# Hunger-Prevails/3D-Pose-Estimation-with-Previleged-Information

Measured on AMD Instinct MI355X. Metric: crops/sec (fwd+bwd) ResNet-50 pose head, 256x256 bs=64/GPU, higher is better.
Workload: dtype f32 (3xbf16 split, 6 products, f32 accumulate); 1 GPU; depthnet resnet50 pose head, 256x256 crops, batch 64/GPU, full step: fwd + soft-argmax + SmoothL1 + bwd + RCCL grad all-reduce + clip + Adam; global_batch=64, parallelism=dp1, dist_world_size=1, wgrad_stream_runs_beside_launch_stream=True

## Files before the change

3d-pose-estimation-with-previleged-information_amd/_lib.py:

```python
import ctypes
import os

_HERE = os.path.dirname(os.path.abspath(__file__))
LIB_PATH = os.environ.get('P3D_LIB') or os.path.join(_HERE, 'csrc', 'libp3d_hip.so')
HEADER_PATH = os.path.join(os.path.dirname(_HERE), 'include', 'p3d_hip.h')


class P3DError(RuntimeError):
    pass


class ConvDesc(ctypes.Structure):
    _fields_ = [(n, ctypes.c_int32) for n in
                ('N', 'C', 'H', 'W', 'K', 'R', 'S', 'stride', 'pad', 'dil', 'Ho', 'Wo', 'c_total', 'c_offset',
                 'accumulate', 'reserved')]


class FoldJob(ctypes.Structure):
    _fields_ = [(n, ctypes.c_void_p) for n in ('w', 'conv_bias', 'gamma', 'beta', 'mean', 'var', 'out', 'bias_out')] + \
               [(n, ctypes.c_int32) for n in ('K', 'C', 'RS', 'c_offset', 'c_total', 'kind')] + [('eps', ctypes.c_float), ('reserved', ctypes.c_int32)]


_i32, _i64, _f32 = ctypes.c_int32, ctypes.c_int64, ctypes.c_float
_ptr, _sz = ctypes.c_void_p, ctypes.c_size_t
# ... 25 lines not shown
    'p3d_fx_conv_fwd_infer_supported': (_i32, [_desc, _i32]),
    'p3d_fx_conv_fwd_infer_workspace_bytes': (_sz, [_desc]),
    'p3d_fx_conv_fwd_infer': (_i32, [_desc, _ptr, _ptr, _ptr, _sz, _ptr, _ptr, _i32, _ptr, _ptr, _sz, _ptr]),
    'p3d_fx_conv_fwd_infer_masked_supported': (_i32, [_desc]),
    'p3d_fx_conv_fwd_infer_masked': (_i32, [_desc, _ptr, _ptr, _sz, _ptr, _ptr, _ptr, _ptr, _i32, _ptr, _ptr, _sz, _ptr]),
    'p3d_stem_tail_infer': (_i32, [_ptr, _ptr, _ptr, _i32, _i32, _i32, _i32, _ptr]),
    'p3d_hblock_workspace_bytes': (_i32, [_ptr, _ptr, _ptr]),
    'p3d_hblock_fwd': (_i32, [_ptr, _ptr, _ptr, _sz, _ptr]),
    'p3d_hblock_bwd': (_i32, [_ptr, _ptr, _ptr, _sz, _ptr, _sz, _ptr, _ptr]),
    'p3d_fx_act_image_bytes': (_sz, [_i32, _i32, _i32]),
    'p3d_fx_act_image': (_i32, [_i32, _ptr, _ptr, _ptr, _i32, _ptr, _i32, _i32, _i32, _ptr]),
    'p3d_fx_conv_img_workspace_bytes': (_sz, [_ptr, _i32]),
    'p3d_fx_conv_img_supported': (_i32, [_ptr]),
    'p3d_fx_conv_fwd_img': (_i32, [_ptr, _ptr, _ptr, _ptr, _ptr, _ptr, _ptr, _sz, _ptr]),
    'p3d_fx_conv_dgrad_img': (_i32, [_ptr, _ptr, _ptr, _ptr, _ptr, _ptr, _sz, _ptr]),
    'p3d_fx_conv_wgrad_img': (_i32, [_ptr, _ptr, _ptr, _ptr, _ptr, _ptr, _sz, _ptr]),
    'p3d_stem_supported': (_i32, [_i32] * 5),
    'p3d_stem_image_bytes': (_sz, [_i32] * 3),
    'p3d_stem_weight_image_bytes': (_sz, [_i32]),
    'p3d_stem_workspace_bytes': (_sz, [_i32] * 4),
    'p3d_stem_image': (_i32, [_ptr, _ptr, _i32, _i32, _i32, _i32, _ptr]),
    'p3d_stem_weight_image': (_i32, [_ptr, _i32, _i32, _ptr, _ptr, _sz, _ptr]),
    'p3d_stem_fwd': (_i32, [_ptr, _ptr, _ptr, _i32, _i32, _i32, _i32, _i32, _ptr]),
    'p3d_stem_wgrad': (_i32, [_ptr, _ptr, _ptr, _i32, _i32, _i32, _i32, _i32, _i32, _ptr, _sz, _ptr]),
    'p3d_stem_masked_supported': (_i32, [_i32] * 5),
    'p3d_stem_image_masked': (_i32, [_ptr, _ptr, _ptr, _i32, _i32, _i32, _i32, _ptr]),
    'p3d_stem_fwd_masked': (_i32, [_ptr, _ptr, _ptr, _ptr, _i32, _i32, _i32, _i32, _i32, _ptr]),
    'p3d_stem_wgrad_masked': (_i32, [_ptr, _ptr, _ptr, _ptr, _i32, _i32, _i32, _i32, _i32, _i32, _ptr, _sz, _ptr]),
    'p3d_profile_enable': (_i32, [_i32]),
    'p3d_profile_collect': (_i32, [ctypes.POINTER(ctypes.c_double), ctypes.POINTER(ctypes.c_double), ctypes.POINTER(ctypes.c_int64)]),
# ... 96 lines not shown
```

3d-pose-estimation-with-previleged-information_amd/csrc/p3d_block.hip:

```cpp
#include "p3d_common.h"
#include "p3d_fx.h"
#include <vector>
#include <mutex>

namespace p3d {

using f32x4 = float __attribute__((ext_vector_type(4)));

constexpr int CLOSE_MAX_SPLIT = 64;
constexpr int FIN_CH = 16, FIN_MAX_LANES = 64;
static inline unsigned fin_threads(int rows) { return rows > 64 ? 1024u : 256u; }
constexpr int BLOCK_MIN_M = 64;
static bool block_conv_ok(const p3d_conv_desc* d, bool main_chain) {
    return fx_fwd_applies(d, BLOCK_MIN_M) && fx_dgrad_applies(d, BLOCK_MIN_M) && fx_wgrad_applies(d, BLOCK_MIN_M) && (d->Ho * d->Wo) % 4 == 0 &&
           (d->H * d->W) % 4 == 0 && d->C % 16 == 0 && d->K % 16 == 0 && !(main_chain && fx_dgrad_has_dead_classes(d));
}

__device__ __forceinline__ void blk_sum3(double& a, double& b, double& c, double* red ) {
    a = wave_sum(a); b = wave_sum(b); c = wave_sum(c);
    const int w = threadIdx.x >> 6;
    if ((threadIdx.x & 63) == 0) { red[w] = a; red[4 + w] = b; red[8 + w] = c; }
    __syncthreads();
    a = red[0] + red[1] + red[2] + red[3];
    b = red[4] + red[5] + red[6] + red[7];
// ... 798 lines not shown
}

int32_t p3d_fx_conv_dgrad_img(const p3d_conv_desc* d, const void* dy_img, const float* w, const void* wimgT, float* dx, void* workspace, size_t workspace_bytes,
                              void* stream) {
    P3D_REQUIRE(d && dy_img && w && dx, "fx_conv_dgrad_img: null argument");
    P3D_REQUIRE(fx_dgrad_applies(d, 32) && d->K % 16 == 0 && (d->Ho * d->Wo) % 4 == 0, "fx_conv_dgrad_img: shape outside the x3 kernels");
    FxFuse f{};
    f.act_img = dy_img; f.wimg = wimgT;
    ProfScope ps(1, d, (hipStream_t)stream);
    fx_count(1, d);
    if (fx_dgrad_has_dead_classes(d) && !d->accumulate)
        if (hipMemsetAsync(dx, 0, (size_t)d->N * d->C * d->H * d->W * sizeof(float), (hipStream_t)stream) != hipSuccess) { set_error("fx_conv_dgrad_img: memset failed"); return P3D_ELAUNCH; }
    return fx_conv_dgrad(d, nullptr, w, dx, workspace, workspace_bytes, &f, (hipStream_t)stream);
}

int32_t p3d_fx_conv_wgrad_img(const p3d_conv_desc* d, const void* dy_img, const float* x, const void* x_img, float* dw, void* workspace, size_t workspace_bytes,
                              void* stream) {
    P3D_REQUIRE(d && dy_img && (x || x_img) && dw, "fx_conv_wgrad_img: null argument");
    P3D_REQUIRE(fx_wgrad_applies(d, 32) && d->K % 16 == 0 && (!x_img || d->C % 16 == 0), "fx_conv_wgrad_img: shape outside the x3 kernels");
    const int splits = fx_wgrad_splits(d, x_img != nullptr);
    const size_t need = (size_t)splits * d->K * d->C * d->R * d->S * sizeof(float);
    if (!workspace || workspace_bytes < need) { set_error("fx_conv_wgrad_img: workspace %zu B < required %zu B", workspace_bytes, need); return P3D_EWORKSPACE; }
    FxFuse f{};
    f.dy_img = dy_img; f.x_img = x_img;
    ProfScope ps(2, d, (hipStream_t)stream);
    fx_count(2, d);
    if (int32_t e = fx_conv_wgrad_slabs(d, nullptr, x, (float*)workspace, splits, &f, (hipStream_t)stream)) return e;
    return wgrad_finish(d, (float*)workspace, splits, d->R * d->S > 1, dw, (hipStream_t)stream);
}

// ... 144 lines not shown
```

3d-pose-estimation-with-previleged-information_amd/csrc/p3d_fx.hip:

```cpp
#include <type_traits>
#include <mutex>
#include "p3d_common.h"
#include "p3d_fx.h"

namespace p3d {

using bf8 = __bf16 __attribute__((ext_vector_type(8)));
using f32x16 = float __attribute__((ext_vector_type(16)));
using f32x4 = float __attribute__((ext_vector_type(4)));
using f32x2 = float __attribute__((ext_vector_type(2)));
using u32x2 = unsigned __attribute__((ext_vector_type(2)));
using s4t = short __attribute__((ext_vector_type(4)));
using s8v = short __attribute__((ext_vector_type(8)));
using i32x4 = int __attribute__((ext_vector_type(4)));

constexpr int FX_BM = 128, FX_BN = 128, FX_BK = 16;
constexpr int FX_PIECE = 128 * FX_BK * 2;

using bf16x2 = __bf16 __attribute__((ext_vector_type(2)));
__device__ __forceinline__ unsigned fx_pack2(float a, float b) {
    const bf16x2 h = __builtin_convertvector(f32x2{a, b}, bf16x2);
    return __builtin_bit_cast(unsigned, h);
}
__device__ __forceinline__ void fx_split2(float x0, float x1, unsigned& hp, unsigned& mp, unsigned& lp) {
// ... 68 lines not shown
        const int row = 8 * (g >> 1) + 4 * half + q;
        off[half] = fx_tr_off(row, ((cb + 16 * (g & 1)) >> 3) + (pq >> 1)) + 8 * (pq & 1);
    }
}

__device__ __forceinline__ FxConvParams fx_class_params(const FxConvParams& in) {
    FxConvParams p = in;
    if (in.ncls > 0) {
        const FxConvClass& c = in.cls[blockIdx.z];
        p.nR = c.nR; p.nS = c.nS; p.ntap = c.ntap; p.r0 = c.r0; p.rstep = c.rstep; p.s0 = c.s0; p.sstep = c.sstep;
        p.hoff = c.hoff; p.hstep = c.hstep; p.woff = c.woff; p.wstep = c.wstep; p.oy0 = c.oy0; p.ox0 = c.ox0;
    }
    return p;
}

template <int AMODE, int PRO, int EPIX, bool TAPI = false>
__global__ __launch_bounds__(256, 3) void fx_conv_kernel(const FxConvParams p_in) {
    static_assert(!TAPI || AMODE == 1, "the tap-inner K order is an image-fed instance");
    constexpr int EPI = EPIX == 5 ? 1 : EPIX == 6 ? 2 : EPIX == 7 || EPIX == 8 || EPIX == 9 ? 0 : EPIX;
    constexpr bool EM = EPIX == 4 || (EPIX >= 5 && EPIX <= 7);
    const FxConvParams p = fx_class_params(p_in);
    static_assert(AMODE == 0 || PRO == 0, "the partial-convolution factor is applied by the in-kernel split");
    __shared__ __attribute__((aligned(16))) unsigned char lds[2 * 6 * FX_PIECE];
    constexpr int BUFB = 6 * FX_PIECE, CH0 = 3 * FX_PIECE;
    float (*const red)[2][128] = reinterpret_cast<float (*)[2][128]>(lds + 40960);
    const int t = threadIdx.x, lane = t & 63, wave = __builtin_amdgcn_readfirstlane(t >> 6), wm = wave >> 1, wn = wave & 1;
    int bid;
    {
        const int nwg = gridDim.x, q = nwg >> 3, r = nwg & 7, xcd = blockIdx.x & 7, idx = blockIdx.x >> 3;
        bid = (xcd < r ? xcd * (q + 1) : r * (q + 1) + (xcd - r) * q) + idx;
    }
    const int tiles_n_all = gridDim.x / p.tiles_m;
    const int tile_m = p.order ? bid / tiles_n_all : bid % p.tiles_m, tile_n = p.order ? bid % tiles_n_all : bid / p.tiles_m;
    const int m0 = tile_m * FX_BM, n0 = tile_n * FX_BN;
    const int OHW = p.OH * p.OW;
    const int HWi = p.Hi * p.Wi;
    const int nfirst = n0 / OHW;
    const int csteps = p.Cred / FX_BK;
    int nk = p.ntap * csteps, kt0 = 0;
    if (p.kchunk > 0) {
        kt0 = blockIdx.y * p.kchunk;
        nk = min(nk - kt0, p.kchunk);
    }
    int f_tap = kt0 / csteps, f_k = (kt0 - f_tap * csteps) * FX_BK;
    if constexpr (TAPI) { f_k = (kt0 / p.ntap) * FX_BK; f_tap = kt0 - (kt0 / p.ntap) * p.ntap; }

    const i32x4 rW = fx_rsrc(p.Wimg, (size_t)p.R * p.S * p.tiles_m * csteps * (3 * FX_PIECE));
    int w_voff[3];
#pragma unroll
    for (int j = 0; j < 3; ++j) w_voff[j] = 16 * (t + 256 * j);

    const int trow = t >> 5, tp4 = t & 31;
    const int pp = t >> 1, ph = (t & 1) ^ ((t >> 4) & 1);
    const int col = n0 + (AMODE == 0 ? 4 * tp4 : pp);
    const bool col_ok = col < p.NP;
    int hbase = 0, wbase = 0, img_off = 0, mimg_off = 0;
    {
        const int cc = col_ok ? col : 0;
        const int pn = cc / OHW;
        const int rem = cc - pn * OHW, oh = rem / p.OW, ow = rem - oh * p.OW;
        hbase = oh * p.hmul + p.hoff;
        wbase = ow * p.wmul + p.woff;
        img_off = AMODE == 0 ? ((pn - nfirst) * p.Cred + trow) * HWi : (pn - nfirst) * csteps * HWi;
        mimg_off = (pn - nfirst) * HWi;
    }
// ... 36 lines not shown
#pragma unroll
                    for (int e = 0; e < 4; ++e) tmask[e] = fx_buffer_load_f32(rPM, x_voff[e] >= 0 ? mbase + e * p.wmul * 4 : FX_OOB, 0, 0);
                }
            }
        }
    };

    f32x4 rx[2];
    i32x4 rwi[3], rxi[3];
    f32x4 smask = {1.f, 1.f, 1.f, 1.f};
    auto fetch = [&]() {
        if (f_tap != cur_tap) { asm volatile("" ::: "memory"); set_tap(f_tap); }
        {
            const int so = w_tapoff + (f_k >> 4) * (3 * FX_PIECE);
#pragma unroll
            for (int j = 0; j < 3; ++j) rwi[j] = fx_buffer_load_i32x4(rW, w_voff[j], FX_SO(so), 0);
        }
        if constexpr (AMODE != 0) {
            const int so = (f_k >> 4) * HWi * 32;
#pragma unroll
            for (int pc = 0; pc < 3; ++pc) rxi[pc] = fx_buffer_load_i32x4(rXi[pc], x_voff[0], FX_SO(so), 0);
        } else {
#pragma unroll
            for (int i = 0; i < 2; ++i) {
                const int so = (f_k + 8 * i) * HWi * 4;
                if (x_vec) rx[i] = fx_buffer_load_f32x4(rX, x_voff[0], FX_SO(so), 0);
                else {
#pragma unroll
                    for (int e = 0; e < 4; ++e) rx[i][e] = fx_buffer_load_f32(rX, x_voff[e], FX_SO(so), 0);
                }
            }
            if constexpr (PRO == 4) smask = tmask;
        }
        if constexpr (TAPI) { if (++f_tap == p.ntap) { f_tap = 0; f_k += FX_BK; } }
        else {
            f_k += FX_BK;
            if (f_k == p.Cred) { f_k = 0; ++f_tap; }
        }
    };
    const int st_p[2] = {fx_tr_off(trow, tp4 >> 1) + 8 * (tp4 & 1), fx_tr_off(trow + 8, tp4 >> 1) + 8 * (tp4 & 1)};
    const int st_p1 = fx_rc_off(pp, ph);
    auto stage = [&](int buf) {
        unsigned char* pb = lds + buf * BUFB;
        unsigned char* cb = pb + CH0;
#pragma unroll
        for (int j = 0; j < 3; ++j) *reinterpret_cast<i32x4*>(cb + 16 * (t + 256 * j)) = rwi[j];
        if constexpr (AMODE != 0) {
#pragma unroll
            for (int pc = 0; pc < 3; ++pc) *reinterpret_cast<i32x4*>(pb + pc * FX_PIECE + st_p1) = rxi[pc];
        } else {
#pragma unroll
            for (int i = 0; i < 2; ++i) {
                f32x4 v = rx[i];
                if constexpr (PRO == 4) {
#pragma unroll
                    for (int e = 0; e < 4; ++e) v[e] *= smask[e];
                }
                fx_split_store(pb + st_p[i], v);
            }
        }
    };

    f32x16 acc[2][2];
#pragma unroll
// ... 10 lines not shown
        else rd_p[a][0] = rd_p[a][1] = fx_rc_off(wn * 64 + a * 32 + fr, fh);
        rd_c[a] = CH0 + fx_rc_off(wm * 64 + a * 32 + fr, fh);
    }
    const int live_b = fx_live_subtiles(m0 + wm * 64, p.M);
    if (nk > 0) { fetch(); stage(0); if (nk > 1) fetch(); }
    __syncthreads();
    auto kloop = [&](auto nbt) {
        constexpr int NB = decltype(nbt)::value;
        bf8 pf[3][2], cf[3][2];
        auto step = [&](int kt, auto st, auto fe) {
            const int buf = kt & 1;
            const unsigned char* bb = lds + buf * BUFB;
            auto read_p = [&](int pc) {
#pragma unroll
                for (int a = 0; a < 2; ++a) {
                    if constexpr (AMODE == 0) pf[pc][a] = fx_tr_read(bb + pc * FX_PIECE, rd_p[a]);
                    else pf[pc][a] = *reinterpret_cast<const bf8*>(bb + pc * FX_PIECE + rd_p[a][0]);
                }
            };
            auto read_c = [&](int pc) {
#pragma unroll
                for (int a = 0; a < 2; ++a)
                    if (a < NB) cf[pc][a] = *reinterpret_cast<const bf8*>(bb + pc * FX_PIECE + rd_c[a]);
            };
            if constexpr (NB > 0) {
                if (FX_ABL_READ(kt)) { read_p(2); read_c(0); read_p(0); read_c(2); }
                __builtin_amdgcn_sched_barrier(0);
                P3D_FX_PRODUCTS_RANGE(acc, pf, cf, 2, NB, 0, 1)
                __builtin_amdgcn_sched_barrier(0);
            }
#ifndef P3D_FX_ABL_NOSTAGE
            if constexpr (decltype(st)::value) stage(buf ^ 1);
// ... 123 lines not shown
                    }
                }
                if constexpr (EPI == 2) {
                    if (!split) {
                        const f32x4 c2 = *reinterpret_cast<const f32x4*>(p.ep_c + ((size_t)n * p.M + m) * OHW + rem);
#pragma unroll
                        for (int e = 0; e < 4; ++e) {
                            const float gg = fmaf(c2[e], esc[b], esh[b]) > 0.f ? v[e] : 0.f;
                            ssum[b] += gg; ssq[b] = fmaf(gg, c2[e] - emean[b], ssq[b]);
                        }
                    }
                }
            }
        }
    if (dense) {
        constexpr int EROW = 512 + 16;
        const bool accum = EPI != 3 && !split && p.accumulate;
#pragma unroll
        for (int b = 0; b < 2; ++b) {
            if (b == 1) __syncthreads();
#pragma unroll
            for (int a = 0; a < 2; ++a)
#pragma unroll
                for (int g = 0; g < 4; ++g)
                    *reinterpret_cast<f32x4*>(lds + (wm * 32 + fr) * EROW + (wn * 64 + a * 32 + 8 * g + 4 * fh) * 4) =
                        f32x4{acc[a][b][4 * g], acc[a][b][4 * g + 1], acc[a][b][4 * g + 2], acc[a][b][4 * g + 3]};
            __syncthreads();
#pragma unroll
            for (int i = 0; i < 8; ++i) {
                const int id = t + 256 * i, row = id >> 5, q = id & 31;
                const int m = m0 + (row >> 5) * 64 + b * 32 + (row & 31);
                const int c4 = n0 + 4 * q;
                if (m >= p.M || c4 >= p.NP) continue;
                const int n = c4 / OHW, rem = c4 - n * OHW;
                f32x4 v = *reinterpret_cast<const f32x4*>(lds + row * EROW + q * 16);
                const size_t at = ((size_t)n * p.M + m) * OHW + rem;
                f32x4* dst = reinterpret_cast<f32x4*>(yout + at);
                if (accum) {
                    f32x4 o4;
                    if (p.acc_src) {
                        o4 = *reinterpret_cast<const f32x4*>(p.acc_src + at);
                        if (p.acc_mask) {
                            const unsigned mk = p.acc_mask[at >> 2];
#pragma unroll
                            for (int e = 0; e < 4; ++e) o4[e] = (mk >> e) & 1u ? o4[e] : 0.f;
// ... 11 lines not shown
                    if (p.ep_relu) { v[0] = fmaxf(v[0], 0.f); v[1] = fmaxf(v[1], 0.f); v[2] = fmaxf(v[2], 0.f); v[3] = fmaxf(v[3], 0.f); }
                }
                *dst = v;
            }
        }
    }
    if constexpr (EPI == 1 || EPI == 2) {
        if (!split) {
#pragma unroll
            for (int b = 0; b < 2; ++b) {
                ssum[b] += __shfl_xor(ssum[b], 32, 64);
                ssq[b] += __shfl_xor(ssq[b], 32, 64);
                if (fh == 0) { red[wn][0][wm * 64 + b * 32 + fr] = ssum[b]; red[wn][1][wm * 64 + b * 32 + fr] = ssq[b]; }
            }
            __syncthreads();
            if (t < 128 && m0 + t < p.M) {
                float* dst = p.partial + ((size_t)tile_n * p.M + m0 + t) * 2;
                dst[0] = red[0][0][t] + red[1][0][t];
                dst[1] = red[0][1][t] + red[1][1][t];
            }
        }
    }
    if constexpr (EPI == 3) {
        float (*const red3)[3][128] = reinterpret_cast<float (*)[3][128]>(lds + 40960);
#pragma unroll
        for (int b = 0; b < 2; ++b) {
            ssum[b] += __shfl_xor(ssum[b], 32, 64);
            ssq[b] += __shfl_xor(ssq[b], 32, 64);
            sthird[b] += __shfl_xor(sthird[b], 32, 64);
            if (fh == 0) { const int ch = wm * 64 + b * 32 + fr; red3[wn][0][ch] = ssum[b]; red3[wn][1][ch] = ssq[b]; red3[wn][2][ch] = sthird[b]; }
        }
        __syncthreads();
        if (t < 128 && m0 + t < p.M)
            *reinterpret_cast<f32x4*>(p.tail_partial + ((size_t)tile_n * p.M + m0 + t) * 4) =
                f32x4{red3[0][0][t] + red3[1][0][t], red3[0][1][t] + red3[1][1][t], red3[0][2][t] + red3[1][2][t], 0.f};
    }
}

template <int BM, int EPI, bool TAPI = false>
__global__ __launch_bounds__(256, 3) void fx16_conv_kernel(const FxConvParams p_in) {
    const FxConvParams p = fx_class_params(p_in);
    static_assert(BM == 128 || BM == 96 || BM == 64, "channel tile");
    constexpr int GA = 4, GB = BM / 32;
    constexpr int WCH = BM / 2;
    constexpr int PIECE_P = 128 * 32, PIECE_C = BM * 32;
    constexpr int BUFB = 3 * PIECE_P + 3 * PIECE_C, CH0 = 3 * PIECE_P;
    constexpr int LDSB = 2 * BUFB > 43008 ? 2 * BUFB : 43008;
    __shared__ __attribute__((aligned(16))) unsigned char lds[LDSB];
    float (*const red)[2][128] = reinterpret_cast<float (*)[2][128]>(lds + 40960);
    const int t = threadIdx.x, lane = t & 63, wave = __builtin_amdgcn_readfirstlane(t >> 6), wm = wave >> 1, wn = wave & 1;
// ... 938 lines not shown
static int g_class_launches = 0;
static int g_fx16 = -1;
static int fx16_mode() {
    if (g_fx16 < 0) { const char* e = getenv("P3D_FX16"); g_fx16 = e ? atoi(e) : 1; if (g_fx16 < 0 || g_fx16 > 2) g_fx16 = 1; }
    return g_fx16;
}
static int fx16_bm(int M, bool img, int pro, int epi) {
    const int mode = fx16_mode();
    if (epi == 5 || epi == 6 || epi == 7) epi = epi == 7 ? 0 : epi - 4;
    if (epi == 8) epi = 0;
    if (!img || pro != 0 || (epi != 0 && epi != 1 && epi != 2) || mode == 0) return 0;
    if (M <= 64) return 64;
    if (ceil_div(M, 96) * 96 < ceil_div(M, 128) * 128) return 96;
    return mode == 2 ? 128 : 0;
}
void fx_tune(int what, int value) {
    if (what == 3) { g_pair_map = value; return; }
    if (what == 5) { g_class_launches = value ? 1 : 0; return; }
    if (what == 9) { g_two_taps = value < 0 ? 1 : value; return; }
    if (what == 10) { g_tap_inner_min = value; return; }
    if (what == 7) { g_conv_order = value; return; }
    if (what == 8) { g_wgrad_order = value; return; }
    if (what == 4) { g_fx16 = value < 0 || value > 2 ? 1 : value; return; }
    (what == 0 ? g_force_wgrad_splits : what == 1 ? g_force_conv_splits : g_wgrad_target) = value;
}

struct FxSplit { int splits, kchunk; };
static FxSplit fx_plan_split(int64_t tiles, int nk) {
    FxSplit s{1, 0};
    int64_t want;
    if (g_force_conv_splits > 0) want = g_force_conv_splits < nk ? g_force_conv_splits : nk;
// ... 147 lines not shown
    if (njobs <= 0) return P3D_OK;
    hipLaunchKernelGGL(fx_fold_bn_kernel, dim3((unsigned)(blocks < 1 ? 1 : blocks), (unsigned)njobs), dim3(256), 0, st, (const p3d_fold_job*)jobs);
    return check_launch("fx_fold_bn_images");
}

int32_t fx_build_weight_images(const float* w, int K, int C, int RS, void* img_fwd, void* img_bwd, hipStream_t st, int ctot, int coff) {
    if (ctot <= 0) { ctot = C; coff = 0; }
    const size_t a = img_fwd ? fx_weight_image_bytes(K, C, RS, false) / 48 : 0, b = img_bwd ? fx_weight_image_bytes(K, C, RS, true) / 48 : 0;
    const size_t total = a > b ? a : b;
    if (total == 0) return P3D_OK;
    const unsigned blocks = (unsigned)(ceil_div((int64_t)total, 256) < 4096 ? ceil_div((int64_t)total, 256) : 4096);
    hipLaunchKernelGGL(fx_weight_images_kernel, dim3(blocks, 2), dim3(256), 0, st, w, (unsigned char*)img_fwd, (unsigned char*)img_bwd, K, C, RS, ctot, coff);
    return check_launch("fx_build_weight_images");
}

static void fx_launch_conv(const FxConvParams& p_in, bool img, int pro, int epi, int bm, dim3 grid, hipStream_t st) {
    const int am = img ? 1 : 0;
    FxConvParams p = p_in;
    if (p.tap_inner && !((bm == 0 && am == 1 && pro == 0 && epi >= 0 && epi <= 2) || (bm == 96 && epi >= 0 && epi <= 2))) p.tap_inner = 0;
    if (p.tap_inner) {
#define P3D_FX_TAPI(EPI) if (bm == 0 && epi == EPI) { hipLaunchKernelGGL((fx_conv_kernel<1, 0, EPI, true>), grid, dim3(256), 0, st, p); return; } \
                         if (bm == 96 && epi == EPI) { hipLaunchKernelGGL((fx16_conv_kernel<96, EPI, true>), grid, dim3(256), 0, st, p); return; }
        P3D_FX_TAPI(0) P3D_FX_TAPI(1) P3D_FX_TAPI(2)
#undef P3D_FX_TAPI
    }
#define P3D_FX16_CASE(BM, EPI) if (bm == BM && (epi == EPI || epi == (EPI == 0 ? 7 : EPI + 4))) { hipLaunchKernelGGL((fx16_conv_kernel<BM, EPI>), grid, dim3(256), 0, st, p); return; }
    P3D_FX16_CASE(128, 0) P3D_FX16_CASE(128, 1) P3D_FX16_CASE(128, 2)
    P3D_FX16_CASE(96, 0) P3D_FX16_CASE(96, 1) P3D_FX16_CASE(96, 2)
    P3D_FX16_CASE(64, 0) P3D_FX16_CASE(64, 1) P3D_FX16_CASE(64, 2)
    P3D_FX16_CASE(128, 8) P3D_FX16_CASE(96, 8) P3D_FX16_CASE(64, 8)
#undef P3D_FX16_CASE
#define P3D_FX_CASE(AM, PRO, EPI) if (am == AM && pro == PRO && epi == EPI) { hipLaunchKernelGGL((fx_conv_kernel<AM, PRO, EPI>), grid, dim3(256), 0, st, p); return; }
    P3D_FX_CASE(0, 0, 0) P3D_FX_CASE(0, 0, 1) P3D_FX_CASE(0, 0, 2) P3D_FX_CASE(0, 4, 0) P3D_FX_CASE(0, 4, 4) P3D_FX_CASE(0, 4, 5)
    P3D_FX_CASE(1, 0, 0) P3D_FX_CASE(1, 0, 1) P3D_FX_CASE(1, 0, 2) P3D_FX_CASE(1, 0, 3) P3D_FX_CASE(1, 0, 5) P3D_FX_CASE(1, 0, 6) P3D_FX_CASE(1, 0, 7)
// ... 52 lines not shown
    }
    const int tiles_n = (int)ceil_div(p.NP, FX_BN);
    const FxSplit sp = fx_fwd_split(d);
    const int bm = fx16_bm(d->K, img, sp.splits > 1 ? 0 : pro, sp.splits > 1 ? 0 : epi);
    p.tiles_m = (int)ceil_div(d->K, bm ? bm : FX_BM);
    p.order = fx_conv_order(fx_weight_image_bytes(d->K, d->C, RS, false), p.tiles_m, tiles_n);
    p.tap_inner = img && RS > 1 && g_tap_inner_min > 0 && d->C >= g_tap_inner_min;
    if (sp.splits > 1) {
        p.kchunk = sp.kchunk; p.slab_stride = (size_t)d->N * d->K * d->Ho * d->Wo; p.Y = (float*)ws; p.bias = nullptr;
        const float* em = p.emask;
        p.emask = nullptr;
        fx_launch_conv(p, img, pro == 4 ? 4 : 0, 0, bm, dim3((unsigned)(p.tiles_m * tiles_n), (unsigned)sp.splits), st);
        fx_launch_reduce(epi, dim3((unsigned)d->K, (unsigned)(d->N < 16 ? d->N : 16)), st, (const float*)ws, y, bias, sp.splits, p.slab_stride, d->N, d->K,
                         d->Ho * d->Wo, d->accumulate, nullptr, nullptr, p.partial, em, p.ep_res, p.ep_relu);
    } else {
        fx_launch_conv(p, img, pro, epi, bm, dim3((unsigned)(p.tiles_m * tiles_n), 1), st);
    }
    return check_launch("fx_conv_fwd");
}

int32_t fx_conv_dgrad(const p3d_conv_desc* d, const float* dy, const float* w, float* dx, void* workspace, size_t workspace_bytes, const FxFuse* fuse,
                      hipStream_t st) {
    const bool img = fuse && fuse->act_img;
    const bool masked = fuse && (fuse->pmask || fuse->emask);
    const void* wimg = fuse ? fuse->wimg : nullptr;
    P3D_REQUIRE(!wimg || (d->c_offset == 0 && d->c_total == d->C), "fx_conv_dgrad: a cached weight image with a channel window (c_offset %d, c_total %d, C %d)",
                d->c_offset, d->c_total, d->C);
    if (masked && (!fuse->emask || (img ? fuse->pmask != nullptr : fuse->pmask == nullptr) || (!img && fuse->partial))) {
        set_error("fx_conv_dgrad: the partial-convolution instances take the result factor and the operand factor exactly for an fp32 operand"); return P3D_EINVAL;
    }
    const size_t need = fx_dgrad_workspace(d);
// ... 38 lines not shown
        p.OH = d->H; p.OW = d->W; p.NP = d->N * d->H * d->W; p.oy0 = 0; p.ox0 = 0; p.oys = 1; p.oxs = 1;
        p.nR = d->R; p.nS = d->S; p.ntap = RS; p.r0 = 0; p.rstep = 1; p.s0 = 0; p.sstep = 1;
        p.hmul = 1; p.hoff = d->pad; p.hstep = -d->dil; p.wmul = 1; p.woff = d->pad; p.wstep = -d->dil;
        const int tiles_n = (int)ceil_div(p.NP, FX_BN);
        const FxSplit sp = fx_dgrad_split(d);
        p.order = fx_conv_order(fx_weight_image_bytes(d->K, d->C, RS, true), p.tiles_m, tiles_n);
        if (sp.splits > 1) {
            p.kchunk = sp.kchunk; p.slab_stride = (size_t)d->N * d->C * d->H * d->W; p.Y = (float*)ws;
            const float* em = p.emask;
            p.emask = nullptr;
            fx_launch_conv(p, img, pro == 4 ? 4 : 0, 0, bm, dim3((unsigned)(p.tiles_m * tiles_n), (unsigned)sp.splits), st);
            fx_launch_reduce(epi, dim3((unsigned)d->C, (unsigned)(d->N < 16 ? d->N : 16)), st, (const float*)ws, dx, nullptr, sp.splits, p.slab_stride, d->N, d->C,
                             d->H * d->W, d->accumulate, p.ep_c, p.ep_tab, p.partial, em);
        } else {
            if (fuse && fuse->acc_src && d->accumulate) { p.acc_src = fuse->acc_src; p.acc_mask = fuse->acc_mask; }
            fx_launch_conv(p, img, pro, epi, bm, dim3((unsigned)(p.tiles_m * tiles_n), 1), st);
        }
        return check_launch("fx_conv_dgrad");
    }
    if (epi != 0 && epi != 4 && epi != 7) { set_error("fx_conv_dgrad: the BatchNorm-backward epilogue is not available for strided data gradients"); return P3D_EINVAL; }
    const int st2 = d->stride;
    p.OH = d->H / st2; p.OW = d->W / st2; p.NP = d->N * p.OH * p.OW; p.oys = st2; p.oxs = st2;
    p.hmul = 1; p.wmul = 1;
    const int tiles_n = (int)ceil_div(p.NP, FX_BN);
    FxConvClass cls[4];
    int ncls = 0;
    for (int ph = 0; ph < st2; ++ph)
        for (int pw = 0; pw < st2; ++pw) {
            int nr = 0, ns = 0, r0 = -1, r1 = -1, q0 = -1, q1 = -1;
            for (int r = 0; r < d->R; ++r) { const int tt = ph + d->pad - r * d->dil; if (((tt % st2) + st2) % st2 == 0) { if (r0 < 0) r0 = r; else if (r1 < 0) r1 = r; ++nr; } }
            for (int s = 0; s < d->S; ++s) { const int tt = pw + d->pad - s * d->dil; if (((tt % st2) + st2) % st2 == 0) { if (q0 < 0) q0 = s; else if (q1 < 0) q1 = s; ++ns; } }
            if (nr == 0 || ns == 0) continue;
            FxConvParams c = p;
            c.nR = nr; c.nS = ns; c.ntap = nr * ns; c.r0 = r0; c.rstep = r1 < 0 ? 1 : r1 - r0; c.s0 = q0; c.sstep = q1 < 0 ? 1 : q1 - q0;
            const int th = ph + d->pad - r0 * d->dil, tw = pw + d->pad - q0 * d->dil;
            c.hoff = th >= 0 ? th / st2 : -((-th) / st2); c.hstep = -(c.rstep * d->dil) / st2;
            c.woff = tw >= 0 ? tw / st2 : -((-tw) / st2); c.wstep = -(c.sstep * d->dil) / st2;
            c.oy0 = ph; c.ox0 = pw;
            if (g_class_launches) { fx_launch_conv(c, img, pro, epi, bm, dim3((unsigned)(c.tiles_m * tiles_n), 1), st); continue; }
            cls[ncls++] = FxConvClass{c.nR, c.nS, c.ntap, c.r0, c.rstep, c.s0, c.sstep, c.hoff, c.hstep, c.woff, c.wstep, c.oy0, c.ox0};
        }
    if (ncls > 0) {
        for (int i = 1; i < ncls; ++i)
            for (int j = i; j > 0 && cls[j].ntap > cls[j - 1].ntap; --j) { const FxConvClass t = cls[j]; cls[j] = cls[j - 1]; cls[j - 1] = t; }
        p.ncls = ncls;
        for (int i = 0; i < ncls; ++i) p.cls[i] = cls[i];
        fx_launch_conv(p, img, pro, epi, bm, dim3((unsigned)(p.tiles_m * tiles_n), 1, (unsigned)ncls), st);
    }
    return check_launch("fx_conv_dgrad");
}

bool fx_dgrad_tail_applies(const p3d_conv_desc* d) {
    return fx_dgrad_applies(d, 96) && d->stride == 1 && fx_dgrad_split(d).splits == 1 && (d->H * d->W) % 4 == 0 && fx16_bm(d->C, true, 0, 0) == 0;
}
int fx_dgrad_tail_rows(const p3d_conv_desc* d) { return (int)ceil_div((int64_t)d->N * d->H * d->W, FX_BN); }
__global__ __launch_bounds__(64) void fx_tail_fold_kernel(const float* __restrict__ partial, int rows, int C, double* __restrict__ sums, int out_rows) {
    const int c = blockIdx.x * 64 + threadIdx.x, r = blockIdx.y;
    if (c >= C) return;
    double s0 = 0.0, s1 = 0.0, s2 = 0.0;
    for (int i = r; i < rows; i += out_rows) {
        const f32x4 v = *reinterpret_cast<const f32x4*>(partial + ((size_t)i * C + c) * 4);
        s0 += v[0]; s1 += v[1]; s2 += v[2];
// ... 225 lines not shown
```

include/p3d_hip.h:

```cpp
#ifndef P3D_HIP_H
#define P3D_HIP_H

#include <stdint.h>
#include <stddef.h>

#ifdef __cplusplus
extern "C" {
#endif

#define P3D_OK 0
#define P3D_EINVAL (-1)
#define P3D_EWORKSPACE (-2)
#define P3D_ELAUNCH (-3)

#define P3D_VERSION 100

int32_t p3d_version(void);
const char* p3d_last_error(void);
int32_t p3d_stream_create(int32_t priority_class, void** stream);
int32_t p3d_stream_create_beside(void* main_stream, void** stream, int32_t* overlaps);
int32_t p3d_stream_create_cumask(const uint32_t* mask, int32_t words, void** stream);
int32_t p3d_probe_hw_ids(void* stream, int32_t* out_device, int32_t nblocks, int32_t spin_us);
int32_t p3d_stream_destroy(void* stream);

// ... 119 lines not shown

int32_t p3d_fx_weight_image_bytes(int32_t K, int32_t C, int32_t RS, size_t* fwd_bytes, size_t* bwd_bytes);
int32_t p3d_fx_weight_images(const float* w, int32_t K, int32_t C, int32_t RS, void* img_fwd, void* img_bwd, void* stream);
int32_t p3d_fx_weight_images_batched(const void* jobs, int32_t njobs, int32_t blocks, void* stream);

size_t p3d_fx_act_image_bytes(int32_t N, int32_t C, int32_t HW);
int32_t p3d_fx_act_image(int32_t mode, const float* x, const float* x2, const float* table, int32_t masked, void* img, int32_t N, int32_t C, int32_t HW, void* stream);
size_t p3d_fx_conv_img_workspace_bytes(const p3d_conv_desc* d, int32_t pass);
int32_t p3d_fx_conv_img_supported(const p3d_conv_desc* d);
int32_t p3d_fx_conv_fwd_img(const p3d_conv_desc* d, const void* x_img, const float* w, const void* wimg, const float* bias, float* y, void* workspace,
                            size_t workspace_bytes, void* stream);
int32_t p3d_fx_conv_dgrad_img(const p3d_conv_desc* d, const void* dy_img, const float* w, const void* wimgT, float* dx, void* workspace, size_t workspace_bytes,
                              void* stream);
int32_t p3d_fx_conv_wgrad_img(const p3d_conv_desc* d, const void* dy_img, const float* x, const void* x_img, float* dw, void* workspace, size_t workspace_bytes,
                              void* stream);

typedef struct p3d_fold_job {
    const float* w;
    const float* conv_bias;
    const float* gamma;
    const float* beta;
    const float* mean;
    const float* var;
    void* out;
    float* bias_out;
    int32_t K, C, RS, c_offset, c_total, kind;
    float eps;
    int32_t reserved;
} p3d_fold_job;
int32_t p3d_fx_fold_bn_images(const void* jobs, int32_t njobs, int32_t blocks, void* stream);
// ... 152 lines not shown
```

Before: 2303 crops/s.

## Add wide 512-thread conv tile doubling N per workgroup for deep-K image-fed convs

Adds a WIDE instance of the image-fed conv kernel that uses 8 waves (4 along N), doubling the N tile per workgroup. Each weight tile loaded into LDS is then reused across twice as many output columns. It is enabled by default for unsplit plain/BN-epilogue forward and dgrad convs where C*taps is at least 1024 and at least the row count. The epilogue partial-sum layout is generalized to the wider tile. The trade-off is one workgroup per CU, a larger LDS footprint and fewer workgroups in the grid, which can reduce occupancy and latency hiding. It also adds test-facing entry points for the partial-sum kernels.

New measurement: 2295 crops/s (median of 2 runs). About the same (-0.3%).

```diff
diff --git a/3d-pose-estimation-with-previleged-information_amd/_lib.py b/3d-pose-estimation-with-previleged-information_amd/_lib.py
--- a/3d-pose-estimation-with-previleged-information_amd/_lib.py
+++ b/3d-pose-estimation-with-previleged-information_amd/_lib.py
@@ -63,6 +63,8 @@
     'p3d_fx_conv_img_supported': (_i32, [_ptr]),
     'p3d_fx_conv_fwd_img': (_i32, [_ptr, _ptr, _ptr, _ptr, _ptr, _ptr, _ptr, _sz, _ptr]),
     'p3d_fx_conv_dgrad_img': (_i32, [_ptr, _ptr, _ptr, _ptr, _ptr, _ptr, _sz, _ptr]),
+    'p3d_fx_conv_img_sums': (_i32, [_ptr, _i32, _ptr, _ptr, _ptr, _ptr, _ptr, _ptr, _ptr, _ptr, _sz, _ptr]),
+    'p3d_fx_conv_img_partial_rows': (_i32, [_ptr, _i32]),
     'p3d_fx_conv_wgrad_img': (_i32, [_ptr, _ptr, _ptr, _ptr, _ptr, _ptr, _sz, _ptr]),
     'p3d_stem_supported': (_i32, [_i32] * 5),
     'p3d_stem_image_bytes': (_sz, [_i32] * 3),
diff --git a/3d-pose-estimation-with-previleged-information_amd/csrc/p3d_block.hip b/3d-pose-estimation-with-previleged-information_amd/csrc/p3d_block.hip
--- a/3d-pose-estimation-with-previleged-information_amd/csrc/p3d_block.hip
+++ b/3d-pose-estimation-with-previleged-information_amd/csrc/p3d_block.hip
@@ -836,6 +836,26 @@
     return fx_conv_dgrad(d, nullptr, w, dx, workspace, workspace_bytes, &f, (hipStream_t)stream);
 }
 
+int32_t p3d_fx_conv_img_sums(const p3d_conv_desc* d, int32_t pass, const void* act_img, const float* w, const void* wimg, float* out, float* partial,
+                             const float* ep_c, const float* ep_tab, void* workspace, size_t workspace_bytes, void* stream) {
+    P3D_REQUIRE(d && act_img && w && out && partial && (pass == 0 || (pass == 1 && ep_c && ep_tab)), "fx_conv_img_sums: null argument or pass %d", pass);
+    FxFuse f{};
+    f.act_img = act_img; f.wimg = wimg; f.partial = partial;
+    if (pass == 0) {
+        P3D_REQUIRE(fx_fwd_applies(d, 32) && d->C % 16 == 0 && (d->H * d->W) % 4 == 0, "fx_conv_img_sums: shape outside the x3 kernels");
+        fx_count(0, d);
+        return fx_conv_fwd(d, nullptr, w, nullptr, out, workspace, workspace_bytes, &f, (hipStream_t)stream);
+    }
+    P3D_REQUIRE(fx_dgrad_applies(d, 32) && d->stride == 1 && d->K % 16 == 0 && (d->Ho * d->Wo) % 4 == 0, "fx_conv_img_sums: shape outside the x3 kernels");
+    f.ep_c = ep_c; f.ep_tab = ep_tab;
+    fx_count(1, d);
+    return fx_conv_dgrad(d, nullptr, w, out, workspace, workspace_bytes, &f, (hipStream_t)stream);
+}
+int32_t p3d_fx_conv_img_partial_rows(const p3d_conv_desc* d, int32_t pass) {
+    if (!d || (pass != 0 && pass != 1)) return 0;
+    return pass == 0 ? fx_partial_rows_fwd(d) : fx_partial_rows_dgrad(d);
+}
+
 int32_t p3d_fx_conv_wgrad_img(const p3d_conv_desc* d, const void* dy_img, const float* x, const void* x_img, float* dw, void* workspace, size_t workspace_bytes,
                               void* stream) {
     P3D_REQUIRE(d && dy_img && (x || x_img) && dw, "fx_conv_wgrad_img: null argument");
diff --git a/3d-pose-estimation-with-previleged-information_amd/csrc/p3d_fx.hip b/3d-pose-estimation-with-previleged-information_amd/csrc/p3d_fx.hip
--- a/3d-pose-estimation-with-previleged-information_amd/csrc/p3d_fx.hip
+++ b/3d-pose-estimation-with-previleged-information_amd/csrc/p3d_fx.hip
@@ -106,17 +106,25 @@
     return p;
 }
 
-template <int AMODE, int PRO, int EPIX, bool TAPI = false>
-__global__ __launch_bounds__(256, 3) void fx_conv_kernel(const FxConvParams p_in) {
+template <int AMODE, int PRO, int EPIX, bool TAPI = false, bool WIDE = false>
+__global__ __launch_bounds__(WIDE ? 512 : 256, WIDE ? 1 : 3) void fx_conv_kernel(const FxConvParams p_in) {
     static_assert(!TAPI || AMODE == 1, "the tap-inner K order is an image-fed instance");
+    static_assert(!WIDE || (AMODE == 1 && PRO == 0 && EPIX <= 3), "the wide tile is an image-fed instance of the plain / BatchNorm epilogues");
     constexpr int EPI = EPIX == 5 ? 1 : EPIX == 6 ? 2 : EPIX == 7 || EPIX == 8 || EPIX == 9 ? 0 : EPIX;
     constexpr bool EM = EPIX == 4 || (EPIX >= 5 && EPIX <= 7);
     const FxConvParams p = fx_class_params(p_in);
     static_assert(AMODE == 0 || PRO == 0, "the partial-convolution factor is applied by the in-kernel split");
-    __shared__ __attribute__((aligned(16))) unsigned char lds[2 * 6 * FX_PIECE];
-    constexpr int BUFB = 6 * FX_PIECE, CH0 = 3 * FX_PIECE;
-    float (*const red)[2][128] = reinterpret_cast<float (*)[2][128]>(lds + 40960);
-    const int t = threadIdx.x, lane = t & 63, wave = __builtin_amdgcn_readfirstlane(t >> 6), wm = wave >> 1, wn = wave & 1;
+    constexpr int WN = WIDE ? 4 : 2;
+    constexpr int NT = 128 * WN, BNP = 64 * WN;
+    constexpr int PIECE_P = BNP * FX_BK * 2;
+    constexpr int EROW = 4 * BNP + 16;
+    constexpr int BUFB = 3 * PIECE_P + 3 * FX_PIECE, CH0 = 3 * PIECE_P;
+    constexpr int RED0 = WIDE ? 64 * EROW : 40960;
+    constexpr int LDSB = 2 * BUFB;
+    static_assert(64 * EROW <= RED0 && RED0 + WN * 3 * 128 * 4 <= LDSB, "LDS layout of the epilogue");
+    __shared__ __attribute__((aligned(16))) unsigned char lds[LDSB];
+    float (*const red)[2][128] = reinterpret_cast<float (*)[2][128]>(lds + RED0);
+    const int t = threadIdx.x, lane = t & 63, wave = __builtin_amdgcn_readfirstlane(t >> 6), wm = wave / WN, wn = wave % WN;
     int bid;
     {
         const int nwg = gridDim.x, q = nwg >> 3, r = nwg & 7, xcd = blockIdx.x & 7, idx = blockIdx.x >> 3;
@@ -124,7 +132,7 @@
     }
     const int tiles_n_all = gridDim.x / p.tiles_m;
     const int tile_m = p.order ? bid / tiles_n_all : bid % p.tiles_m, tile_n = p.order ? bid % tiles_n_all : bid / p.tiles_m;
-    const int m0 = tile_m * FX_BM, n0 = tile_n * FX_BN;
+    const int m0 = tile_m * FX_BM, n0 = tile_n * BNP;
     const int OHW = p.OH * p.OW;
     const int HWi = p.Hi * p.Wi;
     const int nfirst = n0 / OHW;
@@ -138,9 +146,11 @@
     if constexpr (TAPI) { f_k = (kt0 / p.ntap) * FX_BK; f_tap = kt0 - (kt0 / p.ntap) * p.ntap; }
 
     const i32x4 rW = fx_rsrc(p.Wimg, (size_t)p.R * p.S * p.tiles_m * csteps * (3 * FX_PIECE));
+    constexpr int WCH = WIDE ? 2 : 3;
+    const bool w_all = !WIDE || wave < 4;
     int w_voff[3];
 #pragma unroll
-    for (int j = 0; j < 3; ++j) w_voff[j] = 16 * (t + 256 * j);
+    for (int j = 0; j < 3; ++j) w_voff[j] = 16 * (t + NT * j);
 
     const int trow = t >> 5, tp4 = t & 31;
     const int pp = t >> 1, ph = (t & 1) ^ ((t >> 4) & 1);
@@ -207,7 +217,8 @@
         {
             const int so = w_tapoff + (f_k >> 4) * (3 * FX_PIECE);
 #pragma unroll
-            for (int j = 0; j < 3; ++j) rwi[j] = fx_buffer_load_i32x4(rW, w_voff[j], FX_SO(so), 0);
+            for (int j = 0; j < WCH; ++j)
+                if (j < WCH - 1 || w_all) rwi[j] = fx_buffer_load_i32x4(rW, w_voff[j], FX_SO(so), 0);
         }
         if constexpr (AMODE != 0) {
             const int so = (f_k >> 4) * HWi * 32;
@@ -237,10 +248,11 @@
         unsigned char* pb = lds + buf * BUFB;
         unsigned char* cb = pb + CH0;
 #pragma unroll
-        for (int j = 0; j < 3; ++j) *reinterpret_cast<i32x4*>(cb + 16 * (t + 256 * j)) = rwi[j];
+        for (int j = 0; j < WCH; ++j)
+            if (j < WCH - 1 || w_all) *reinterpret_cast<i32x4*>(cb + 16 * (t + NT * j)) = rwi[j];
         if constexpr (AMODE != 0) {
 #pragma unroll
-            for (int pc = 0; pc < 3; ++pc) *reinterpret_cast<i32x4*>(pb + pc * FX_PIECE + st_p1) = rxi[pc];
+            for (int pc = 0; pc < 3; ++pc) *reinterpret_cast<i32x4*>(pb + pc * PIECE_P + st_p1) = rxi[pc];
         } else {
 #pragma unroll
             for (int i = 0; i < 2; ++i) {
@@ -281,8 +293,8 @@
             auto read_p = [&](int pc) {
 #pragma unroll
                 for (int a = 0; a < 2; ++a) {
-                    if constexpr (AMODE == 0) pf[pc][a] = fx_tr_read(bb + pc * FX_PIECE, rd_p[a]);
-                    else pf[pc][a] = *reinterpret_cast<const bf8*>(bb + pc * FX_PIECE + rd_p[a][0]);
+                    if constexpr (AMODE == 0) pf[pc][a] = fx_tr_read(bb + pc * PIECE_P, rd_p[a]);
+                    else pf[pc][a] = *reinterpret_cast<const bf8*>(bb + pc * PIECE_P + rd_p[a][0]);
                 }
             };
             auto read_c = [&](int pc) {
@@ -436,7 +448,6 @@
             }
         }
     if (dense) {
-        constexpr int EROW = 512 + 16;
         const bool accum = EPI != 3 && !split && p.accumulate;
 #pragma unroll
         for (int b = 0; b < 2; ++b) {
@@ -450,7 +461,7 @@
             __syncthreads();
 #pragma unroll
             for (int i = 0; i < 8; ++i) {
-                const int id = t + 256 * i, row = id >> 5, q = id & 31;
+                const int id = t + NT * i, row = id / (BNP / 4), q = id % (BNP / 4);
                 const int m = m0 + (row >> 5) * 64 + b * 32 + (row & 31);
                 const int c4 = n0 + 4 * q;
                 if (m >= p.M || c4 >= p.NP) continue;
@@ -492,15 +503,16 @@
                 if (fh == 0) { red[wn][0][wm * 64 + b * 32 + fr] = ssum[b]; red[wn][1][wm * 64 + b * 32 + fr] = ssq[b]; }
             }
             __syncthreads();
-            if (t < 128 && m0 + t < p.M) {
-                float* dst = p.partial + ((size_t)tile_n * p.M + m0 + t) * 2;
-                dst[0] = red[0][0][t] + red[1][0][t];
-                dst[1] = red[0][1][t] + red[1][1][t];
+            const int h = t >> 7, c = t & 127, row = tile_n * (WN / 2) + h;
+            if (t < 64 * WN && m0 + c < p.M && row * 128 < p.NP) {
+                float* dst = p.partial + ((size_t)row * p.M + m0 + c) * 2;
+                dst[0] = red[2 * h][0][c] + red[2 * h + 1][0][c];
+                dst[1] = red[2 * h][1][c] + red[2 * h + 1][1][c];
             }
         }
     }
     if constexpr (EPI == 3) {
-        float (*const red3)[3][128] = reinterpret_cast<float (*)[3][128]>(lds + 40960);
+        float (*const red3)[3][128] = reinterpret_cast<float (*)[3][128]>(lds + RED0);
 #pragma unroll
         for (int b = 0; b < 2; ++b) {
             ssum[b] += __shfl_xor(ssum[b], 32, 64);
@@ -509,9 +521,10 @@
             if (fh == 0) { const int ch = wm * 64 + b * 32 + fr; red3[wn][0][ch] = ssum[b]; red3[wn][1][ch] = ssq[b]; red3[wn][2][ch] = sthird[b]; }
         }
         __syncthreads();
-        if (t < 128 && m0 + t < p.M)
-            *reinterpret_cast<f32x4*>(p.tail_partial + ((size_t)tile_n * p.M + m0 + t) * 4) =
-                f32x4{red3[0][0][t] + red3[1][0][t], red3[0][1][t] + red3[1][1][t], red3[0][2][t] + red3[1][2][t], 0.f};
+        const int h = t >> 7, c = t & 127, row = tile_n * (WN / 2) + h;
+        if (t < 64 * WN && m0 + c < p.M && row * 128 < p.NP)
+            *reinterpret_cast<f32x4*>(p.tail_partial + ((size_t)row * p.M + m0 + c) * 4) =
+                f32x4{red3[2 * h][0][c] + red3[2 * h + 1][0][c], red3[2 * h][1][c] + red3[2 * h + 1][1][c], red3[2 * h][2][c] + red3[2 * h + 1][2][c], 0.f};
     }
 }
 
@@ -1480,7 +1493,21 @@
     if (ceil_div(M, 96) * 96 < ceil_div(M, 128) * 128) return 96;
     return mode == 2 ? 128 : 0;
 }
+static int g_wide = -1;
+static int fx_wide_mode() {
+    if (g_wide < 0) { const char* e = getenv("P3D_FX_WIDE"); g_wide = e ? atoi(e) : 1; if (g_wide < 0 || g_wide > 2) g_wide = 1; }
+    return g_wide;
+}
+static bool fx_wide_tile(int rows, int cred, int ntap, bool img, int pro, int epi, int bm, bool split) {
+    if (!img || pro != 0 || bm != 0 || split || epi < 0 || epi > 3) return false;
+    const int mode = fx_wide_mode();
+    if (mode == 0) return false;
+    if (mode == 2) return true;
+    const int64_t k = (int64_t)cred * ntap;
+    return k >= 1024 && k >= rows;
+}
 void fx_tune(int what, int value) {
+    if (what == 11) { g_wide = value < 0 || value > 2 ? 1 : value; return; }
     if (what == 3) { g_pair_map = value; return; }
     if (what == 5) { g_class_launches = value ? 1 : 0; return; }
     if (what == 9) { g_two_taps = value < 0 ? 1 : value; return; }
@@ -1658,10 +1685,20 @@
     return check_launch("fx_build_weight_images");
 }
 
-static void fx_launch_conv(const FxConvParams& p_in, bool img, int pro, int epi, int bm, dim3 grid, hipStream_t st) {
+static void fx_launch_conv(const FxConvParams& p_in, bool img, int pro, int epi, int bm, dim3 grid, hipStream_t st, bool wide = false) {
     const int am = img ? 1 : 0;
     FxConvParams p = p_in;
     if (p.tap_inner && !((bm == 0 && am == 1 && pro == 0 && epi >= 0 && epi <= 2) || (bm == 96 && epi >= 0 && epi <= 2))) p.tap_inner = 0;
+    if (wide) {
+#define P3D_FX_WIDE(EPI) if (epi == EPI) { if (p.tap_inner) hipLaunchKernelGGL((fx_conv_kernel<1, 0, EPI, true, true>), grid, dim3(512), 0, st, p); \
+                                           else hipLaunchKernelGGL((fx_conv_kernel<1, 0, EPI, false, true>), grid, dim3(512), 0, st, p); return; }
+        if (am == 1 && pro == 0 && bm == 0) {
+            P3D_FX_WIDE(0) P3D_FX_WIDE(1) P3D_FX_WIDE(2)
+            if (epi == 3) { hipLaunchKernelGGL((fx_conv_kernel<1, 0, 3, false, true>), grid, dim3(512), 0, st, p); return; }
+        }
+#undef P3D_FX_WIDE
+        set_error("fx_launch_conv: no wide-tile instance for img=%d pro=%d epi=%d bm=%d tap_inner=%d", am, pro, epi, bm, p.tap_inner); return;
+    }
     if (p.tap_inner) {
 #define P3D_FX_TAPI(EPI) if (bm == 0 && epi == EPI) { hipLaunchKernelGGL((fx_conv_kernel<1, 0, EPI, true>), grid, dim3(256), 0, st, p); return; } \
                          if (bm == 96 && epi == EPI) { hipLaunchKernelGGL((fx16_conv_kernel<96, EPI, true>), grid, dim3(256), 0, st, p); return; }
@@ -1744,7 +1781,8 @@
         fx_launch_reduce(epi, dim3((unsigned)d->K, (unsigned)(d->N < 16 ? d->N : 16)), st, (const float*)ws, y, bias, sp.splits, p.slab_stride, d->N, d->K,
                          d->Ho * d->Wo, d->accumulate, nullptr, nullptr, p.partial, em, p.ep_res, p.ep_relu);
     } else {
-        fx_launch_conv(p, img, pro, epi, bm, dim3((unsigned)(p.tiles_m * tiles_n), 1), st);
+        const bool wide = fx_wide_tile(d->K, d->C, RS, img, pro, epi, bm, false);
+        fx_launch_conv(p, img, pro, epi, bm, dim3((unsigned)(p.tiles_m * (wide ? ceil_div(p.NP, 2 * FX_BN) : tiles_n)), 1), st, wide);
     }
     return check_launch("fx_conv_fwd");
 }
@@ -1813,7 +1851,8 @@
                              d->H * d->W, d->accumulate, p.ep_c, p.ep_tab, p.partial, em);
         } else {
             if (fuse && fuse->acc_src && d->accumulate) { p.acc_src = fuse->acc_src; p.acc_mask = fuse->acc_mask; }
-            fx_launch_conv(p, img, pro, epi, bm, dim3((unsigned)(p.tiles_m * tiles_n), 1), st);
+            const bool wide = fx_wide_tile(d->C, d->K, RS, img, pro, epi, bm, false);
+            fx_launch_conv(p, img, pro, epi, bm, dim3((unsigned)(p.tiles_m * (wide ? ceil_div(p.NP, 2 * FX_BN) : tiles_n)), 1), st, wide);
         }
         return check_launch("fx_conv_dgrad");
     }
@@ -1844,7 +1883,8 @@
             for (int j = i; j > 0 && cls[j].ntap > cls[j - 1].ntap; --j) { const FxConvClass t = cls[j]; cls[j] = cls[j - 1]; cls[j - 1] = t; }
         p.ncls = ncls;
         for (int i = 0; i < ncls; ++i) p.cls[i] = cls[i];
-        fx_launch_conv(p, img, pro, epi, bm, dim3((unsigned)(p.tiles_m * tiles_n), 1, (unsigned)ncls), st);
+        const bool wide = fx_wide_tile(d->C, d->K, RS / (st2 * st2), img, pro, epi, bm, false);
+        fx_launch_conv(p, img, pro, epi, bm, dim3((unsigned)(p.tiles_m * (wide ? ceil_div(p.NP, 2 * FX_BN) : tiles_n)), 1, (unsigned)ncls), st, wide);
     }
     return check_launch("fx_conv_dgrad");
 }
diff --git a/include/p3d_hip.h b/include/p3d_hip.h
--- a/include/p3d_hip.h
+++ b/include/p3d_hip.h
@@ -157,6 +157,9 @@
                               void* stream);
 int32_t p3d_fx_conv_wgrad_img(const p3d_conv_desc* d, const void* dy_img, const float* x, const void* x_img, float* dw, void* workspace, size_t workspace_bytes,
                               void* stream);
+int32_t p3d_fx_conv_img_sums(const p3d_conv_desc* d, int32_t pass, const void* act_img, const float* w, const void* wimg, float* out, float* partial,
+                             const float* ep_c, const float* ep_tab, void* workspace, size_t workspace_bytes, void* stream);
+int32_t p3d_fx_conv_img_partial_rows(const p3d_conv_desc* d, int32_t pass);
 
 typedef struct p3d_fold_job {
     const float* w;
```
